# slp-rl/slamkit

Hardware: NVIDIA H100
Metric: speech-tokens/sec (SLAM seq=1024) (higher is better)
Workload: dtype bf16

## Files before the change

### slamkit_b200/csrc/gemm_tcgen05.cu

```cuda
#include "common.cuh"
#include <cudaTypedefs.h>
#include <stdio.h>
#include <mutex>
#include <type_traits>
#include <string.h>
#include <stdlib.h>
#include "kernels.h"
#include "../../include/slamkit_b200.h"

namespace {

constexpr int BM = 128;
constexpr int BK = 64;
constexpr int MMA_K = 16;
constexpr int GEMM_THREADS = 288;


struct GemmParams {
  int M, N, K;
  int batch;
  int a_mode;
  int passes;
  void* C;
  void* C_lo;
  int ldc;
  const void* bias;
  int bias_f32;
  const bf16* residual;
  const bf16* residual_lo;
  int ldr;
  int tiles_m, tiles_n;
  int out_f32;
  int round_before_res;
  int act;
  int col_gin, col_gout;
  int splits;
  float* splitk_ws;
  int tma_store;
  int reg_epi;
  int pdl;
  int sk_units;
  int sk_groups;
  int sk_G;
  int sk_colunits;
  int sk_carry;
  int units, n_groups;
  float* sk_ws;
  uint32_t* sk_flags;
  int epi;
  const bf16* aux;
  int ld_aux;
  const bf16* rope_cos;
  const bf16* rope_sin;
  const int* rope_pos;
  int rope_T, rope_cols, rope_maxpos, rope_rot;
};

template <int BN, int EW = 4>
struct GemmCfg {
  static constexpr int A_BYTES = BM * BK * 2;
  static constexpr int B_ATOMS = (BN + 63) / 64;
  static constexpr int B_BYTES = B_ATOMS * 64 * BK * 2;
  static constexpr int STAGE_BYTES = A_BYTES + B_BYTES;
  static constexpr int STAGES = (BN > 128) ? 4 : (BN > 64 ? 6 : 8);
  static constexpr int STAGING_BYTES = 4 * 2 * 4096;
  static constexpr int BAR_BYTES = 256;
  static constexpr int SMEM_BYTES = STAGES * STAGE_BYTES + STAGING_BYTES + BAR_BYTES + 1024;
  static_assert(BN % 64 == 0 || (BN == 224 && EW == 4), "a 32-column tail chunk only on the 224-wide tile");
  static_assert(STAGES * STAGE_BYTES >= BM * BN * 4, "the parked fp32 accumulator must fit in the stage ring");
  static_assert(SMEM_BYTES <= 227 * 1024, "sm_90 allows 227 KB of shared memory per block");
};

template <int BN>
SK_DEVINL uint32_t acc_chunk_addr(uint32_t base, int row, int chunk) {
  return base + (uint32_t)row * (BN * 4) + (uint32_t)((chunk ^ (row & 7)) << 4);
}
template <int BN>
SK_DEVINL void acc_park(uint32_t base, const float (&d)[BN / 2], int wg, int warp_in_wg, int lane) {
  const int r0 = 64 * wg + 16 * warp_in_wg + (lane >> 2);
#pragma unroll
  for (int j = 0; j < BN / 8; ++j) {
    const int chunk = 2 * j + ((lane & 3) >> 1);
    const uint32_t off = (uint32_t)(lane & 1) * 8u;
    asm volatile("st.shared.v2.f32 [%0], {%1, %2};" ::"r"(acc_chunk_addr<BN>(base, r0, chunk) + off), "f"(d[4 * j]),
                 "f"(d[4 * j + 1]) : "memory");
    asm volatile("st.shared.v2.f32 [%0], {%1, %2};" ::"r"(acc_chunk_addr<BN>(base, r0 + 8, chunk) + off), "f"(d[4 * j + 2]),
                 "f"(d[4 * j + 3]) : "memory");
  }
}
template <int BN>
SK_DEVINL void acc_ld_32x32(uint32_t base, uint32_t ta, uint32_t (&r)[32]) {
  const int row = (int)(ta >> 16) + (int)(threadIdx.x & 31);
  const int c0 = (int)(ta & 0xffffu) >> 2;
#pragma unroll
  for (int i = 0; i < 8; ++i)
    asm volatile("ld.shared.v4.b32 {%0, %1, %2, %3}, [%4];"
                 : "=r"(r[4 * i]), "=r"(r[4 * i + 1]), "=r"(r[4 * i + 2]), "=r"(r[4 * i + 3])
                 : "r"(acc_chunk_addr<BN>(base, row, c0 + i)) : "memory");
}

SK_DEVINL uint32_t staging_addr(uint32_t sbuf, int lane, int j, bool tail) {
  return tail ? sbuf + (uint32_t)lane * 64u + (uint32_t)((j ^ ((lane >> 1) & 3)) << 4)
              : sbuf + (uint32_t)lane * 128u + (uint32_t)((j ^ (lane & 7)) << 4);
}

SK_DEVINL float gelu_erf(float y) {
  const float a = fabsf(y);
  float t;
  asm("rcp.approx.ftz.f32 %0, %1;" : "=f"(t) : "f"(fmaf(0.3275911f * 0.70710678118654752440f, a, 1.0f)));
  float s = fmaf(0.5f * 1.061405429f, t, 0.5f * -1.453152027f);
  s = fmaf(s, t, 0.5f * 1.421413741f);
  s = fmaf(s, t, 0.5f * -0.284496736f);
  s = fmaf(s, t, 0.5f * 0.254829592f);
  const float e = ex2_approx((y * y) * -0.72134752044448170368f);
  return fmaf(-a, (s * t) * e, fmaxf(y, 0.0f));
}

SK_DEVINL float gelu_exact(float x) { return x * 0.5f * (1.0f + erff(x * 0.70710678118654752440f)); }
SK_DEVINL float gelu_exact_grad(float x) {
  const float cdf = 0.5f * (1.0f + erff(x * 0.70710678118654752440f));
  const float pdf = expf(-0.5f * x * x) * 0.39894228040143267794f;
  return cdf + x * pdf;
}

SK_DEVINL void stmatrix_x4(uint32_t addr, uint32_t a, uint32_t b, uint32_t c, uint32_t d) {
  asm volatile("stmatrix.sync.aligned.m8n8.x4.shared.b16 [%0], {%1, %2, %3, %4};" ::"r"(addr), "r"(a), "r"(b), "r"(c),
               "r"(d) : "memory");
}

template <bool SK>
struct WorkIter {
  int num_kb, splits, kb_per_split, total_items, tiles_n;
  int G, colunits, carry, units, n_groups, sk_groups, grp, mem;
  long sk_total, sk_cur, sk_end;
  int next_unit, next_item;
  int tile, split, kb_begin, kb_end, role;
  long unit_end_it;
  SK_DEVINL WorkIter(const GemmParams& p, int num_kb_, int kb_per_split_, int total_items_) {
    num_kb = num_kb_;
    splits = p.splits;
    kb_per_split = kb_per_split_;
    total_items = total_items_;
    tiles_n = p.tiles_n;
    G = p.sk_G;
    colunits = p.sk_colunits;
    carry = p.sk_carry;
    units = p.units;
    n_groups = p.n_groups;
    sk_groups = p.sk_groups;
    tile = split = kb_begin = kb_end = role = 0;
    unit_end_it = 0;
    sk_total = sk_cur = sk_end = 0;
    next_item = (int)blockIdx.x;
    next_unit = 0;
    grp = mem = 0;
    if (SK && p.sk_units > 0) {
      grp = (int)blockIdx.x / G;
      mem = (int)blockIdx.x - grp * G;
      next_item = total_items;
      next_unit = grp < n_groups ? p.sk_units + grp : units;
      if (grp < sk_groups) {
        sk_total = (long)p.sk_units * num_kb;
        sk_cur = sk_total * grp / sk_groups;
        sk_end = sk_total * (grp + 1) / sk_groups;
      }
    }
  }
  SK_DEVINL int tile_of(int unit) const { return colunits ? mem * tiles_n + unit : unit * G + mem; }
  SK_DEVINL bool next() {
    if (SK && sk_cur < sk_end && carry) {
      const int unit = (int)((sk_end - 1) / num_kb);
      const long ustart = (long)unit * num_kb;
      const long b = sk_cur > ustart ? sk_cur : ustart;
      kb_begin = (int)(b - ustart);
      kb_end = (int)(sk_end - ustart);
      unit_end_it = ustart + num_kb;
      tile = tile_of(unit);
      split = 0;
      role = kb_begin != 0 ? 3 : (kb_end < num_kb ? 1 : 0);
      sk_end = b;
      return true;
    }
    if (SK && sk_cur < sk_end) {
      const int unit = (int)(sk_cur / num_kb);
      kb_begin = (int)(sk_cur - (long)unit * num_kb);
      unit_end_it = (long)(unit + 1) * num_kb;
      const long e = sk_end < unit_end_it ? sk_end : unit_end_it;
      kb_end = kb_begin + (int)(e - sk_cur);
      tile = tile_of(unit);
      split = 0;
      role = kb_begin != 0 ? 1 : (e < unit_end_it ? 2 : 0);
      sk_cur = e;
// ... 746 lines not shown
#pragma unroll
            for (int t = 0; t < 16; ++t) pk[t] = pack_bf16(__uint_as_float(r0[2 * t]), __uint_as_float(r0[2 * t + 1]));
            if constexpr (!tail) {
              acc_ld(taddr + c2 * 64 + 32, r1);
              if (SK && n_contrib > 0) sk_fixup_add(r1, p.sk_ws, c2 * 2 + 1, row_in_tile, first_contrib, w.G, n_contrib);
#pragma unroll
              for (int t = 0; t < 16; ++t) pk[16 + t] = pack_bf16(__uint_as_float(r1[2 * t]), __uint_as_float(r1[2 * t + 1]));
            }
            stage_store(&tmC, pk, n0 + c2 * 64, tail_c);
          });
        } else if (p.tma_store && !p.bias && !p.act && p.residual && !p.residual_lo && p.epi == 0) {
          for_chunks([&](auto tail_c, int c2) {
            constexpr bool tail = decltype(tail_c)::value;
            constexpr int nj = tail ? 4 : 8;
            const int col64 = n0 + c2 * 64;
            if (col64 >= p.N) return;
            uint4 rv[8];
            if (row_ok) {
              const bf16* rp = p.residual + row * p.ldr + col64;
#pragma unroll
              for (int j = 0; j < 8; ++j) rv[j] = (j < nj && col64 + 8 * j < p.N) ? ldg128(rp + 8 * j) : make_uint4(0u, 0u, 0u, 0u);
            } else {
#pragma unroll
              for (int j = 0; j < 8; ++j) rv[j] = make_uint4(0u, 0u, 0u, 0u);
            }
            uint32_t r0[32], r1[32], pk[32];
            acc_ld(taddr + c2 * 64, r0);
            if (SK && n_contrib > 0) sk_fixup_add(r0, p.sk_ws, c2 * 2, row_in_tile, first_contrib, w.G, n_contrib);
            if constexpr (!tail) {
              acc_ld(taddr + c2 * 64 + 32, r1);
              if (SK && n_contrib > 0) sk_fixup_add(r1, p.sk_ws, c2 * 2 + 1, row_in_tile, first_contrib, w.G, n_contrib);
            }
#pragma unroll
            for (int j = 0; j < nj; ++j) {
              const uint32_t* r = j < 4 ? r0 + 8 * j : r1 + 8 * (j - 4);
              const uint32_t rw[4] = {rv[j].x, rv[j].y, rv[j].z, rv[j].w};
#pragma unroll
              for (int e = 0; e < 4; ++e) {
                const float2 f = unpack_bf16(rw[e]);
                float a0 = __uint_as_float(r[2 * e]), a1 = __uint_as_float(r[2 * e + 1]);
                if (p.round_before_res) {
                  const float2 t = unpack_bf16(pack_bf16(a0, a1));
                  a0 = t.x; a1 = t.y;
                }
                pk[4 * j + e] = pack_bf16(a0 + f.x, a1 + f.y);
              }
            }
            stage_store(&tmC, pk, col64, tail_c);
          });
        } else if (p.tma_store) {
          for_chunks([&](auto tail_c, int c2) {
            constexpr bool tail = decltype(tail_c)::value;
            const uint32_t sbuf = staging_base + (EW == 4 ? (uint32_t)warp * 8192u + (store_cnt & 1u) * 4096u : (uint32_t)warp * 4096u);
            if (lane == 0) {
              if constexpr (EW == 4) tma_store_wait_read<1>(); else tma_store_wait_read<0>();
            }
            __syncwarp();
#pragma unroll
            for (int half = 0; half < (tail ? 1 : 2); ++half) {
              uint32_t r[32];
              acc_ld(taddr + c2 * 64 + half * 32, r);
              if (SK && n_contrib > 0) sk_fixup_add(r, p.sk_ws, c2 * 2 + half, row_in_tile, first_contrib, w.G, n_contrib);
#pragma unroll
              for (int g = 0; g < 4; ++g) {
                const int col = n0 + c2 * 64 + half * 32 + g * 8;
                float v[8];
#pragma unroll
                for (int i = 0; i < 8; ++i) v[i] = __uint_as_float(r[g * 8 + i]);
                if (col < p.N) {
                  epi_bias_act(v, p, col);
                  if (row_ok) epi_residual(v, p, row, col);
                }
                asm volatile("st.shared.v4.b32 [%0], {%1, %2, %3, %4};" ::"r"(staging_addr(sbuf, lane, half * 4 + g, tail)),
                             "r"(pack_bf16(v[0], v[1])), "r"(pack_bf16(v[2], v[3])), "r"(pack_bf16(v[4], v[5])),
                             "r"(pack_bf16(v[6], v[7]))
                             : "memory");
              }
            }
            fence_proxy_async();
            __syncwarp();
            if (lane == 0) {
              tma_store_2d(tail ? &tmAux : &tmC, sbuf, n0 + c2 * 64, m0 + q * 32);
              tma_store_commit();
            }
            ++store_cnt;
          });
        }
        else
#pragma unroll 1
        for (int c = chalf * (BN / 32 / CS); c < (chalf + 1) * (BN / 32 / CS); ++c) {
          uint32_t r[32];
          acc_ld(taddr + c * 32, r);
          if (SK && n_contrib > 0) sk_fixup_add(r, p.sk_ws, c, row_in_tile, first_contrib, w.G, n_contrib);
          const int col0 = n0 + c * 32;
          if (row_ok && col0 < p.N) {
#pragma unroll
            for (int g = 0; g < 4; ++g) {
              const int col = col0 + g * 8;
              if (col < p.N) {
                float v[8];
#pragma unroll
                for (int i = 0; i < 8; ++i) v[i] = __uint_as_float(r[g * 8 + i]);
                if (p.splits > 1) {
                  float* dst = p.splitk_ws + ((size_t)split_idx * p.M + row_in) * p.N + col;
                  *reinterpret_cast<float4*>(dst) = make_float4(v[0], v[1], v[2], v[3]);
                  *reinterpret_cast<float4*>(dst + 4) = make_float4(v[4], v[5], v[6], v[7]);
                  continue;
                }
                epi_bias_act(v, p, col);
                int ocol = col;
                if (p.col_gin > 0) {
                  const int gi = col / p.col_gin, ci = col - gi * p.col_gin;
                  if (ci >= p.col_gout) continue;
                  ocol = gi * p.col_gout + ci;
                }
                epi_residual(v, p, row, ocol);
                if (p.out_f32) {
                  float* dst = reinterpret_cast<float*>(p.C) + row * p.ldc + ocol;
                  *reinterpret_cast<float4*>(dst) = make_float4(v[0], v[1], v[2], v[3]);
                  *reinterpret_cast<float4*>(dst + 4) = make_float4(v[4], v[5], v[6], v[7]);
                } else {
                  uint4 o;
                  o.x = pack_bf16(v[0], v[1]);
                  o.y = pack_bf16(v[2], v[3]);
                  o.z = pack_bf16(v[4], v[5]);
                  o.w = pack_bf16(v[6], v[7]);
                  stg128(reinterpret_cast<bf16*>(p.C) + row * p.ldc + ocol, o);
                  if (p.C_lo) {
                    const float2 h0 = unpack_bf16(o.x), h1 = unpack_bf16(o.y), h2 = unpack_bf16(o.z), h3 = unpack_bf16(o.w);
                    uint4 l;
                    l.x = pack_bf16(v[0] - h0.x, v[1] - h0.y);
                    l.y = pack_bf16(v[2] - h1.x, v[3] - h1.y);
                    l.z = pack_bf16(v[4] - h2.x, v[5] - h2.y);
                    l.w = pack_bf16(v[6] - h3.x, v[7] - h3.y);
                    stg128(reinterpret_cast<bf16*>(p.C_lo) + row * p.ldc + ocol, l);
                  }
                }
              }
            }
          }
        }
        if (SK && w.role == 2) {
          __syncwarp();
          if (lane == 0)
            for (int i = 0; i < n_contrib; ++i) p.sk_flags[(first_contrib + i * w.G) * 4 + q] = 0u;
        }
      }
      release_acc();
    }
    if ((epi_warp || p.reg_epi) && p.tma_store && lane == 0) tma_store_wait<0>();
  }
}

__global__ void splitk_reduce_kernel(const float* __restrict__ ws, bf16* __restrict__ C, int M, int N, int ldc, int splits,
                                     int accumulate, int round_before_res) {
  griddep_launch();
  griddep_wait();
  const long total = (long)M * N / 8;
  for (long i = blockIdx.x * (long)blockDim.x + threadIdx.x; i < total; i += (long)gridDim.x * blockDim.x) {
    const long e = i * 8;
    const int m = (int)(e / N), n = (int)(e % N);
    float acc[8] = {0, 0, 0, 0, 0, 0, 0, 0};
    for (int s = 0; s < splits; ++s) {
      const float* src = ws + ((size_t)s * M + m) * N + n;
      const float4 a = *reinterpret_cast<const float4*>(src), b = *reinterpret_cast<const float4*>(src + 4);
      acc[0] += a.x; acc[1] += a.y; acc[2] += a.z; acc[3] += a.w;
      acc[4] += b.x; acc[5] += b.y; acc[6] += b.z; acc[7] += b.w;
    }
    bf16* dst = C + (size_t)m * ldc + n;
    if (accumulate) {
      const uint4 o = *reinterpret_cast<const uint4*>(dst);
      const uint32_t ow[4] = {o.x, o.y, o.z, o.w};
#pragma unroll
      for (int k = 0; k < 4; ++k) {
        const float2 f = unpack_bf16(ow[k]);
        acc[2 * k] = (round_before_res ? bf16_round(acc[2 * k]) : acc[2 * k]) + f.x;
        acc[2 * k + 1] = (round_before_res ? bf16_round(acc[2 * k + 1]) : acc[2 * k + 1]) + f.y;
      }
    }
    stg128(dst, make_uint4(pack_bf16(acc[0], acc[1]), pack_bf16(acc[2], acc[3]), pack_bf16(acc[4], acc[5]),
                           pack_bf16(acc[6], acc[7])));
  }
}

PFN_cuTensorMapEncodeTiled_v12000 g_encode = nullptr;
std::once_flag g_encode_once;

void load_encode() {
  void* fn = nullptr;
  cudaDriverEntryPointQueryResult qres;
  cudaError_t e = cudaGetDriverEntryPoint("cuTensorMapEncodeTiled", &fn, cudaEnableDefault, &qres);
  if (e == cudaSuccess && qres == cudaDriverEntryPointSuccess) g_encode = (PFN_cuTensorMapEncodeTiled_v12000)fn;
}

}

int sk_make_tmap_2d(CUtensorMap* out, const void* ptr, int elem_bytes, uint64_t inner, uint64_t outer, uint64_t ld,
                    uint32_t box_inner, uint32_t box_outer) {
  std::call_once(g_encode_once, load_encode);
  SK_REQUIRE(g_encode != nullptr, "cuTensorMapEncodeTiled driver entry point not available");
  SK_REQUIRE((reinterpret_cast<uintptr_t>(ptr) & 15) == 0, "TMA base pointer must be 16-byte aligned");
  SK_REQUIRE((ld * elem_bytes) % 16 == 0, "TMA row pitch must be a multiple of 16 bytes (ld=%llu)",
             (unsigned long long)ld);
  SK_REQUIRE(box_inner * elem_bytes == 128 || box_inner * elem_bytes == 64, "box inner extent must be 128 (or 64) bytes");
  cuuint64_t dims[2] = {inner, outer};
  cuuint64_t strides[1] = {ld * (uint64_t)elem_bytes};
  cuuint32_t box[2] = {box_inner, box_outer};
  cuuint32_t estr[2] = {1, 1};
  CUtensorMapDataType dt = elem_bytes == 2 ? CU_TENSOR_MAP_DATA_TYPE_BFLOAT16 : CU_TENSOR_MAP_DATA_TYPE_FLOAT32;
  CUresult r = g_encode(out, dt, 2, const_cast<void*>(ptr), dims, strides, box, estr, CU_TENSOR_MAP_INTERLEAVE_NONE,
                        box_inner * elem_bytes == 64 ? CU_TENSOR_MAP_SWIZZLE_64B : CU_TENSOR_MAP_SWIZZLE_128B,
                        CU_TENSOR_MAP_L2_PROMOTION_L2_256B,
                        CU_TENSOR_MAP_FLOAT_OOB_FILL_NONE);
  SK_REQUIRE(r == CUDA_SUCCESS, "cuTensorMapEncodeTiled failed with CUresult %d (inner=%llu outer=%llu ld=%llu)", (int)r,
             (unsigned long long)inner, (unsigned long long)outer, (unsigned long long)ld);
  return 0;
}

int sk_make_tmap_3d(CUtensorMap* out, const void* ptr, uint64_t inner, uint64_t rows, uint64_t batch, uint64_t row_stride,
                    uint64_t batch_stride, uint32_t box_rows) {
  std::call_once(g_encode_once, load_encode);
  SK_REQUIRE(g_encode != nullptr, "cuTensorMapEncodeTiled driver entry point not available");
  SK_REQUIRE((reinterpret_cast<uintptr_t>(ptr) & 15) == 0, "TMA base pointer must be 16-byte aligned");
  SK_REQUIRE((row_stride * 2) % 16 == 0 && (batch_stride * 2) % 16 == 0, "TMA strides must be multiples of 16 bytes");
  cuuint64_t dims[3] = {inner, rows, batch};
  cuuint64_t strides[2] = {row_stride * 2, batch_stride * 2};
  cuuint32_t box[3] = {64, box_rows, 1};
  cuuint32_t estr[3] = {1, 1, 1};
  CUresult r = g_encode(out, CU_TENSOR_MAP_DATA_TYPE_BFLOAT16, 3, const_cast<void*>(ptr), dims, strides, box, estr,
                        CU_TENSOR_MAP_INTERLEAVE_NONE, CU_TENSOR_MAP_SWIZZLE_128B, CU_TENSOR_MAP_L2_PROMOTION_L2_256B,
                        CU_TENSOR_MAP_FLOAT_OOB_FILL_NONE);
  SK_REQUIRE(r == CUDA_SUCCESS, "cuTensorMapEncodeTiled(3d) failed with CUresult %d", (int)r);
  return 0;
}

namespace {

template <int BN, bool A_MN, bool B_MN, bool SK, int EW = 4>
int launch_gemm(const CUtensorMap* tm, const GemmParams& p, int grid, cudaStream_t stream) {
  using Cfg = GemmCfg<BN, EW>;
  static bool attr_set = false;
  if (!attr_set) {
    SK_CUDA_CHECK(cudaFuncSetAttribute(gemm_wgmma_kernel<BN, A_MN, B_MN, SK, EW>, cudaFuncAttributeMaxDynamicSharedMemorySize,
                                       Cfg::SMEM_BYTES));
    attr_set = true;
  }
  sk_prof_begin(0, stream);
  cudaError_t lerr = sk_launch_pdl_if(p.pdl != 0, gemm_wgmma_kernel<BN, A_MN, B_MN, SK, EW>, dim3(grid), dim3(GEMM_THREADS), (size_t)Cfg::SMEM_BYTES, stream,
                                   tm[0], tm[1], tm[2], tm[3], tm[4], tm[5], p);
  sk_prof_end(stream);
  SK_CUDA_CHECK(lerr);
  SK_LAUNCH_CHECK();
  return 0;
}

template <int BN, bool SK, int EW = 4>
int dispatch_major(bool a_mn, bool b_mn, const CUtensorMap* tm, const GemmParams& p, int grid, cudaStream_t s) {
  if (!a_mn && !b_mn) return launch_gemm<BN, false, false, SK, EW>(tm, p, grid, s);
  if (!a_mn && b_mn) return launch_gemm<BN, false, true, SK, EW>(tm, p, grid, s);
  if (a_mn && !b_mn) return launch_gemm<BN, true, false, SK, EW>(tm, p, grid, s);
  return launch_gemm<BN, true, true, SK, EW>(tm, p, grid, s);
}

inline int tile_cost(int bn) { return bn >= 256 ? 100 : (bn > 128 ? 61 + (bn - 128) * 39 / 128 : (bn == 128 ? 61 : 54)); }

constexpr size_t SK_FLAG_BYTES = 4096;

}

size_t sk_gemm_ws_min_bytes(void) { return (size_t)sk_num_sms() * SK_SLOT_FLOATS * sizeof(float) + SK_FLAG_BYTES; }

int sk_pick_bn(int M, int N, int force_bn, bool fit_forced, bool fit, bool whole_heads) {
  if (force_bn == 64 || force_bn == 128 || force_bn == 256) return force_bn;
  if (fit_forced && (force_bn == 192 || (force_bn == 224 && !whole_heads))) return force_bn;
  const int nsm = sk_num_sms();
  auto cost = [&](int bn) {
    const long tiles = (long)((M + BM - 1) / BM) * ((N + bn - 1) / bn);
    return ((tiles + nsm - 1) / nsm) * tile_cost(bn);
  };
  int best = 256;
  long best_cost = cost(256);
  for (const int bn : {128, 64}) {
    if (cost(bn) * 100 < best_cost * 75) {
      best_cost = cost(bn);
      best = bn;
    }
  }
  if (best == 256 && fit && N % 256 != 0) {
    for (const int bn : {224, 192}) {
      if (!(whole_heads && bn % 64 != 0) && cost(bn) * 100 < best_cost * 95) {
        best_cost = cost(bn);
        best = bn;
      }
    }
  }
  return best;
}

namespace {

int plan_gemm(const SkGemmEx& g, GemmParams& p, int& BN, int& ew, int& grid) {
  SK_REQUIRE(g.M > 0 && g.N > 0 && g.K > 0 && g.batch >= 1, "gemm: empty problem M=%d N=%d K=%d batch=%d", g.M, g.N, g.K,
             g.batch);
  SK_REQUIRE(g.N % 8 == 0, "gemm: N must be a multiple of 8 (N=%d)", g.N);
  SK_REQUIRE(g.ldc % 8 == 0 && (g.residual == nullptr || g.ldr % 8 == 0), "gemm: ldc/ldr must be multiples of 8");
  SK_REQUIRE((reinterpret_cast<uintptr_t>(g.C) & 15) == 0, "gemm: C must be 16-byte aligned");
  SK_REQUIRE(((reinterpret_cast<uintptr_t>(g.A) | reinterpret_cast<uintptr_t>(g.B) | reinterpret_cast<uintptr_t>(g.A_lo) |
               reinterpret_cast<uintptr_t>(g.B_lo)) & 15) == 0,
             "gemm: A and B must be 16-byte aligned");
  SK_REQUIRE((reinterpret_cast<uintptr_t>(g.bias) & 15) == 0 && (reinterpret_cast<uintptr_t>(g.residual) & 15) == 0,
             "gemm: bias and residual must be 16-byte aligned");
  SK_REQUIRE(g.passes == 1 || (g.passes == 3 && g.A_lo && g.B_lo), "gemm: passes must be 1, or 3 with lo operands");
  SK_REQUIRE(g.act >= 0 && g.act <= 2, "gemm: act must be 0 (none), 1 (GELU) or 2 (ReLU), got %d", g.act);
  const bool use3d = g.a_rows > 0;
  SK_REQUIRE(!use3d || !g.a_mn, "gemm: a batched / windowed A operand must be K-major");
  SK_REQUIRE(g.a_mode == 0 || use3d, "gemm: a_mode 1 needs the 3-D A view");
  SK_REQUIRE(use3d || g.lda >= (g.a_mn ? g.M : g.K), "gemm: lda=%d is smaller than the %s of A", g.lda, g.a_mn ? "M" : "K");
  SK_REQUIRE(g.ldb >= (g.b_mn ? g.N : g.K), "gemm: ldb=%d is smaller than the %s of B", g.ldb, g.b_mn ? "N" : "K");
  if (g.col_gin == 0) {
    const int out_cols = g.epi == 2 ? 2 * g.N : g.N;
    SK_REQUIRE(g.ldc >= out_cols, "gemm: ldc=%d is smaller than the %d output columns", g.ldc, out_cols);
    SK_REQUIRE(g.residual == nullptr || g.ldr >= g.N, "gemm: ldr=%d is smaller than N=%d", g.ldr, g.N);
  }
  const int nsm = sk_num_sms();
  static const int sk_env = [] { const char* e = getenv("SK_STREAMK"); return e ? atoi(e) : 1; }();
  static const int sk_min_idle = [] { const char* e = getenv("SK_STREAMK_MIN_IDLE"); return e ? atoi(e) : 20; }();
  static const int sk_min_kb = [] { const char* e = getenv("SK_STREAMK_MIN_KB"); return e ? atoi(e) : 32; }();
  const bool sk_ok = sk_env != 0 && g.batch == 1 && !use3d && g.passes == 1 && g.a_mode == 0 && g.splitk_ws != nullptr &&
                     g.splitk_ws_bytes >= sk_gemm_ws_min_bytes();
  const size_t ws_data_bytes = g.splitk_ws_bytes > SK_FLAG_BYTES ? g.splitk_ws_bytes - SK_FLAG_BYTES : 0;
  const bool fit = g.passes == 1 && g.batch == 1 && !use3d && g.a_mode == 0 && g.epi != 1 && g.epi != 2 && g.epi != 4 &&
                   g.epi != 5;
  SK_REQUIRE((g.force_bn != 192 && g.force_bn != 224) || (fit && !(g.force_bn == 224 && g.epi == 3)),
             "gemm: force_bn=%d needs a one-pass 2-D problem (and whole 64-column heads for RoPE)", g.force_bn);
  BN = (g.a_mode == 1) ? 64
                       : sk_pick_bn(g.M * g.batch, g.N, (g.epi == 1 || g.epi == 2) ? 256 : g.force_bn, fit,
                                    fit && !sk_ok, g.epi == 3);
  memset(&p, 0, sizeof(p));
  p.M = g.M; p.N = g.N; p.K = g.K;
  p.batch = g.batch;
  p.a_mode = (g.a_mode & 1) | (use3d ? 2 : 0);
  p.passes = g.passes;
  p.C = g.C; p.C_lo = g.C_lo; p.ldc = g.ldc;
  p.bias = g.bias; p.bias_f32 = g.bias_f32;
  p.residual = reinterpret_cast<const bf16*>(g.residual);
  p.residual_lo = reinterpret_cast<const bf16*>(g.residual_lo);
  p.ldr = g.ldr;
  p.tiles_m = (g.M + BM - 1) / BM;
  p.tiles_n = (g.N + BN - 1) / BN;
  p.out_f32 = g.out_f32;
  p.round_before_res = g.round_before_res;
  p.act = g.act;
  p.col_gin = g.col_gin; p.col_gout = g.col_gout;
  p.pdl = g.pdl;
  const long tiles = (long)p.tiles_m * p.tiles_n * g.batch;
  p.splits = 1;
  p.splitk_ws = nullptr;
  const int num_kb = (g.K + BK - 1) / BK;
  static const int splitk_env = [] { const char* e = getenv("SK_SPLITK"); return e ? atoi(e) : 1; }();
  static const int sk_ranges = [] { const char* e = getenv("SK_STREAMK_RANGES"); return e ? atoi(e) : 4; }();
  if (splitk_env && g.splitk_ws && g.batch == 1 && g.passes == 1 && !g.out_f32 && !g.bias && !g.act && !g.C_lo && g.col_gin == 0 &&
      g.epi == 0 &&
      (g.residual == nullptr || g.residual == g.C) && tiles * 2 <= nsm && num_kb >= 16) {
    int sp = (int)(nsm / tiles);
    if (sp > 8) sp = 8;
    if (sp > num_kb / 4) sp = num_kb / 4;
    if ((size_t)sp * g.M * g.N * sizeof(float) > ws_data_bytes) sp = (int)(ws_data_bytes / ((size_t)g.M * g.N * sizeof(float)));
    if (sp >= 2) {
      const int per = (num_kb + sp - 1) / sp;
      sp = (num_kb + per - 1) / per;
    }
    if (sp >= 2) {
      p.splits = sp;
      p.splitk_ws = reinterpret_cast<float*>(g.splitk_ws);
    }
  }
  p.tma_store = (!g.out_f32 && !g.C_lo && g.col_gin == 0 && p.splits == 1 && g.batch == 1 && !use3d && (g.ldc * 2) % 16 == 0)
                    ? 1 : 0;
  p.epi = g.epi;
  p.aux = reinterpret_cast<const bf16*>(g.aux);
  p.ld_aux = g.ld_aux;
  p.rope_cos = reinterpret_cast<const bf16*>(g.rope_cos);
  p.rope_sin = reinterpret_cast<const bf16*>(g.rope_sin);
  p.rope_pos = g.rope_pos;
  p.rope_T = g.rope_T; p.rope_cols = g.rope_cols; p.rope_maxpos = g.rope_maxpos;
  p.rope_rot = g.rope_rot == 0 ? 64 : g.rope_rot;
  if (g.epi == 6) {
    SK_REQUIRE(g.passes == 1 && g.batch == 1 && !use3d && g.residual && g.aux && !g.residual_lo && !g.act && !g.out_f32 &&
                   !g.C_lo && g.col_gin == 0 && g.round_before_res && g.ld_aux >= g.N && g.ld_aux % 8 == 0 &&
                   (reinterpret_cast<uintptr_t>(g.aux) & 15) == 0,
               "gemm: two-residual epilogue needs a plain one-pass bf16 GEMM, both residuals (16-byte aligned, pitch >= N) and "
               "round_before_res");
  } else if (g.epi != 0) {
    SK_REQUIRE(p.tma_store && g.passes == 1 && !g.residual && !g.act && g.splitk_ws == nullptr,
               "gemm: fused epilogue %d needs the plain bf16 TMA-store path (no residual / activation / scratch)", g.epi);
    if (g.epi == 1) {
      SK_REQUIRE(BN == 256 && g.N % 256 == 0 && g.aux_out && g.ld_aux_out % 8 == 0 && !g.bias,
                 "gemm: SwiGLU-forward epilogue needs N = 2F with F %% 128 == 0 and an act output");
    } else if (g.epi == 2) {
      SK_REQUIRE(BN == 256 && g.N % 128 == 0 && g.aux && g.ld_aux % 8 == 0 && !g.bias,
                 "gemm: SwiGLU-backward epilogue needs N = F with F %% 128 == 0 and the saved gu activation");
    } else if (g.epi == 3) {
      SK_REQUIRE(g.rope_cos && g.rope_sin && g.rope_T > 0 && g.rope_maxpos > 0 && g.rope_cols % 64 == 0 && g.N % 64 == 0 &&
                     !g.bias_f32,
                 "gemm: RoPE epilogue needs cos/sin tables, 64-column heads and a bf16 bias");
      SK_REQUIRE(p.rope_rot == 16 || p.rope_rot == 32 || p.rope_rot == 64,
                 "gemm: RoPE epilogue rotary width rope_rot=%d is not supported (16, 32 or 64)", g.rope_rot);
    } else if (g.epi == 4) {
      SK_REQUIRE(BN % 64 == 0 && g.N % 64 == 0 && g.aux_out && g.ld_aux_out >= g.N && g.ld_aux_out % 8 == 0 && !g.bias_f32 &&
                     (reinterpret_cast<uintptr_t>(g.aux_out) & 15) == 0,
                 "gemm: GELU-forward epilogue needs N %% 64 == 0, an act output (pitch >= N) and a bf16 bias");
    } else if (g.epi == 5) {
      SK_REQUIRE(BN % 64 == 0 && g.N % 64 == 0 && g.aux && g.ld_aux >= g.N && g.ld_aux % 8 == 0 && !g.bias &&
                     (reinterpret_cast<uintptr_t>(g.aux) & 15) == 0,
                 "gemm: GELU-backward epilogue needs N %% 64 == 0, the saved pre-activation (pitch >= N) and no bias");
    } else {
      SK_REQUIRE(false, "gemm: unknown fused epilogue %d", g.epi);
    }
  }
  p.sk_G = 1;
  if (sk_ok && BN == 256 && p.splits == 1 && num_kb >= sk_min_kb && (p.tiles_n <= 8 || p.tiles_m <= 8)) {
    const int colunits = p.tiles_n <= 8 ? 0 : 1;
    const int G = colunits ? p.tiles_m : p.tiles_n;
    const int units = colunits ? p.tiles_n : p.tiles_m;
    const int n_groups = nsm / G;
    const int rem = units % n_groups;
    const long slots = ((long)(units + n_groups - 1) / n_groups) * n_groups;
    const bool multiwave = units > n_groups;
    if (n_groups >= 1 && rem != 0 && (slots - units) * 100 >= slots * sk_min_idle &&
        (!colunits || multiwave || sk_env >= 2)) {
      if (colunits && multiwave) {
        p.sk_units = rem + n_groups;
        p.sk_groups = n_groups;
        p.sk_carry = 1;
      } else {
        p.sk_units = rem;
        p.sk_groups = n_groups < rem * sk_ranges ? n_groups : rem * sk_ranges;
      }
      p.sk_G = G;
      p.sk_colunits = colunits;
      p.units = units;
      p.n_groups = n_groups;
      p.sk_ws = reinterpret_cast<float*>(g.splitk_ws);
      p.sk_flags = reinterpret_cast<uint32_t*>(reinterpret_cast<uint8_t*>(g.splitk_ws) + ws_data_bytes);
    }
  }
  const long work = tiles * p.splits;
  grid = p.sk_units > 0 ? p.n_groups * p.sk_G : (int)(work < nsm ? work : nsm);
  static const int ew_env = [] { const char* e = getenv("SK_GEMM_EW"); return e ? atoi(e) : 0; }();
  ew = (p.sk_units == 0 && BN == 256 && p.tma_store && (ew_env == 8 || (ew_env == 0 && (g.epi == 2 || g.epi == 3 || g.epi == 4 || g.epi == 5)))) ? 8 : 4;
  p.reg_epi = (p.tma_store && p.sk_units == 0 && ew == 4 && !g.bias && !g.act && !g.residual && (g.epi == 0 || g.epi == 1)) ? 1 : 0;
  return 0;
}

}

int sk_gemm_plan_ex(const SkGemmEx& g, SkGemmPlan* out) {
  GemmParams p;
  int BN = 0, ew = 0, grid = 0;
  const int rc = plan_gemm(g, p, BN, ew, grid);
  if (rc) return rc;
  out->bn = BN;
  out->epi_warps = ew;
  out->splits = p.splits;
  out->sk_units = p.sk_units;
  out->sk_groups = p.sk_groups;
  out->sk_G = p.sk_G;
  out->sk_colunits = p.sk_colunits;
  out->tma_store = p.tma_store;
  out->grid = grid;
  return 0;
}

int sk_gemm_ex_launch(const SkGemmEx& g, cudaStream_t stream) {
  GemmParams p;
  int BN = 0, ew = 0, grid = 0;
  const int rc0 = plan_gemm(g, p, BN, ew, grid);
  if (rc0) return rc0;
  const bool use3d = g.a_rows > 0;
  CUtensorMap tm[6];
  const void* As[2] = {g.A, g.passes == 3 ? g.A_lo : g.A};
  const void* Bs[2] = {g.B, g.passes == 3 ? g.B_lo : g.B};
  for (int i = 0; i < 2; ++i) {
    int rc;
    CUtensorMap* ta = &tm[i == 0 ? 0 : 2];
    CUtensorMap* tb = &tm[i == 0 ? 1 : 3];
    if (use3d) {
      rc = sk_make_tmap_3d(ta, As[i], (uint64_t)g.a_inner, (uint64_t)g.a_rows, (uint64_t)g.batch, (uint64_t)g.a_row_stride,
                           (uint64_t)g.a_batch_stride, BM);
    } else if (!g.a_mn) {
      rc = sk_make_tmap_2d(ta, As[i], 2, (uint64_t)g.K, (uint64_t)g.M, (uint64_t)g.lda, BK, BM);
    } else {
      rc = sk_make_tmap_2d(ta, As[i], 2, (uint64_t)g.M, (uint64_t)g.K, (uint64_t)g.lda, 64, BK);
    }
    if (rc) return rc;
    if (!g.b_mn) rc = sk_make_tmap_2d(tb, Bs[i], 2, (uint64_t)g.K, (uint64_t)g.N, (uint64_t)g.ldb, BK, (uint32_t)BN);
    else         rc = sk_make_tmap_2d(tb, Bs[i], 2, (uint64_t)g.N, (uint64_t)g.K, (uint64_t)g.ldb, 64, BK);
    if (rc) return rc;
  }
  tm[4] = tm[0];
  const uint32_t box_rows = p.reg_epi ? 16 : 32;
  if (p.tma_store) {
    const int rc2 = sk_make_tmap_2d(&tm[4], g.C, 2, (uint64_t)(g.epi == 2 ? 2 * g.N : g.N), (uint64_t)g.M, (uint64_t)g.ldc, 64, box_rows);
    if (rc2) return rc2;
  }
  tm[5] = tm[4];
  if (g.epi == 1) {
    const int rc3 = sk_make_tmap_2d(&tm[5], g.aux_out, 2, (uint64_t)g.N / 2, (uint64_t)g.M, (uint64_t)g.ld_aux_out, 64, box_rows);
    if (rc3) return rc3;
  } else if (g.epi == 4) {
    const int rc3 = sk_make_tmap_2d(&tm[5], g.aux_out, 2, (uint64_t)g.N, (uint64_t)g.M, (uint64_t)g.ld_aux_out, 64, 32);
    if (rc3) return rc3;
  } else if (p.tma_store && BN % 64 != 0) {
    const int rc3 = sk_make_tmap_2d(&tm[5], g.C, 2, (uint64_t)g.N, (uint64_t)g.M, (uint64_t)g.ldc, 32, box_rows);
    if (rc3) return rc3;
  }
  int rc;
  if (p.sk_units > 0) {
    rc = dispatch_major<256, true>(g.a_mn, g.b_mn, tm, p, grid, stream);
  } else if (ew == 8) {
    rc = dispatch_major<256, false, 8>(g.a_mn, g.b_mn, tm, p, grid, stream);
  } else {
    switch (BN) {
      case 256: rc = dispatch_major<256, false>(g.a_mn, g.b_mn, tm, p, grid, stream); break;
      case 224: rc = dispatch_major<224, false>(g.a_mn, g.b_mn, tm, p, grid, stream); break;
      case 192: rc = dispatch_major<192, false>(g.a_mn, g.b_mn, tm, p, grid, stream); break;
      case 128: rc = dispatch_major<128, false>(g.a_mn, g.b_mn, tm, p, grid, stream); break;
      default:  rc = dispatch_major<64, false>(g.a_mn, g.b_mn, tm, p, grid, stream); break;
    }
  }
  if (rc) return rc;
  if (p.splits > 1) {
    SK_REQUIRE(g.residual == nullptr || g.residual == g.C, "gemm: split-K supports only in-place accumulation");
    const long n8 = (long)g.M * g.N / 8;
    int blocks = (int)((n8 + 255) / 256);
    if (blocks > sk_num_sms() * 8) blocks = sk_num_sms() * 8;
    sk_prof_begin(0, stream);
    SK_CUDA_CHECK(sk_launch_pdl(splitk_reduce_kernel, dim3(blocks), dim3(256), (size_t)(0), stream, p.splitk_ws, reinterpret_cast<bf16*>(g.C), g.M, g.N, g.ldc, p.splits,
                                                     g.residual != nullptr, g.round_before_res));
    sk_prof_end(stream);
    SK_LAUNCH_CHECK();
  }
  return 0;
}

SkGemmEx sk_gemm_desc(int M, int N, int K, const void* A, int lda, int a_mn, const void* B, int ldb, int b_mn, void* C,
                      int ldc, int out_f32, const void* bias, const void* residual, int ldr, int round_before_res, int act,
                      int force_bn, void* splitk_ws, size_t splitk_ws_bytes) {
  SkGemmEx g;
  memset(&g, 0, sizeof(g));
  g.M = M; g.N = N; g.K = K; g.batch = 1; g.passes = 1;
  g.A = A; g.lda = lda; g.a_mn = a_mn;
  g.B = B; g.ldb = ldb; g.b_mn = b_mn;
  g.C = C; g.ldc = ldc; g.out_f32 = out_f32;
  g.bias = bias; g.residual = residual; g.ldr = ldr; g.round_before_res = round_before_res; g.act = act;
  g.force_bn = force_bn;
  g.pdl = 1;
  g.splitk_ws = splitk_ws;
  g.splitk_ws_bytes = splitk_ws_bytes;
  return g;
}
int sk_gemm_launch(int M, int N, int K, const void* A, int lda, int a_mn, const void* B, int ldb, int b_mn, void* C,
                   int ldc, int out_f32, const void* bias, const void* residual, int ldr, int round_before_res, int act,
                   int force_bn, cudaStream_t stream, void* splitk_ws, size_t splitk_ws_bytes) {
  return sk_gemm_ex_launch(sk_gemm_desc(M, N, K, A, lda, a_mn, B, ldb, b_mn, C, ldc, out_f32, bias, residual, ldr,
                                        round_before_res, act, force_bn, splitk_ws, splitk_ws_bytes),
                           stream);
}

int sk_linear_swiglu_fwd_launch(int M, int F, int K, const void* x, const void* Wgu, void* gu, void* act, cudaStream_t s) {
  SkGemmEx g;
  memset(&g, 0, sizeof(g));
  g.M = M; g.N = 2 * F; g.K = K; g.batch = 1; g.passes = 1;
  g.A = x; g.lda = K; g.B = Wgu; g.ldb = K;
  g.C = gu; g.ldc = 2 * F;
  g.epi = 1; g.aux_out = act; g.ld_aux_out = F;
  g.pdl = 1;
  return sk_gemm_ex_launch(g, s);
}
int sk_linear_swiglu_bwd_launch(int M, int N, int F, const void* dy, const void* Wd, const void* gu, void* dgu, cudaStream_t s) {
  SkGemmEx g;
  memset(&g, 0, sizeof(g));
  g.M = M; g.N = F; g.K = N; g.batch = 1; g.passes = 1;
  g.A = dy; g.lda = N; g.B = Wd; g.ldb = F; g.b_mn = 1;
  g.C = dgu; g.ldc = 2 * F;
  g.epi = 2; g.aux = gu; g.ld_aux = 2 * F;
  g.pdl = 1;
  return sk_gemm_ex_launch(g, s);
}
int sk_linear_rope_launch(int M, int N, int K, const void* x, const void* W, const void* bias, void* out, const void* cos_t,
                          const void* sin_t, const int32_t* pos_ids, int T, int rope_cols, int max_positions, cudaStream_t s,
                          int rope_rot) {
  SkGemmEx g;
  memset(&g, 0, sizeof(g));
  g.M = M; g.N = N; g.K = K; g.batch = 1; g.passes = 1;
  g.A = x; g.lda = K; g.B = W; g.ldb = K;
  g.C = out; g.ldc = N;
  g.bias = bias;
  g.epi = 3; g.rope_cos = cos_t; g.rope_sin = sin_t; g.rope_pos = pos_ids; g.rope_T = T;
  g.rope_cols = rope_cols; g.rope_maxpos = max_positions; g.rope_rot = rope_rot;
  g.pdl = 1;
  return sk_gemm_ex_launch(g, s);
}
int sk_linear_gelu_fwd_launch(int M, int F, int K, const void* x, const void* W1, const void* b1, void* pre, void* act,
                              cudaStream_t s) {
  SkGemmEx g;
  memset(&g, 0, sizeof(g));
  g.M = M; g.N = F; g.K = K; g.batch = 1; g.passes = 1;
  g.A = x; g.lda = K; g.B = W1; g.ldb = K;
  g.C = pre; g.ldc = F;
  g.bias = b1;
  g.epi = 4; g.aux_out = act; g.ld_aux_out = F;
  g.pdl = 1;
  return sk_gemm_ex_launch(g, s);
}
int sk_linear_gelu_bwd_launch(int M, int N, int F, const void* dy, const void* W2, const void* pre, void* dpre, cudaStream_t s) {
  SkGemmEx g;
  memset(&g, 0, sizeof(g));
  g.M = M; g.N = F; g.K = N; g.batch = 1; g.passes = 1;
  g.A = dy; g.lda = N; g.B = W2; g.ldb = F; g.b_mn = 1;
  g.C = dpre; g.ldc = F;
  g.epi = 5; g.aux = pre; g.ld_aux = F;
  g.pdl = 1;
  return sk_gemm_ex_launch(g, s);
}
int sk_linear_res2_launch(int M, int N, int K, const void* x, const void* W, const void* bias, const void* res2, const void* res,
                          void* out, cudaStream_t s, void* splitk_ws, size_t splitk_ws_bytes) {
  SkGemmEx g = sk_gemm_desc(M, N, K, x, K, 0, W, K, 0, out, N, 0, bias, res, N, 1, 0, 0, splitk_ws, splitk_ws_bytes);
  g.epi = 6; g.aux = res2; g.ld_aux = N;
  return sk_gemm_ex_launch(g, s);
}
```

Baseline: 166,600.

## Add warp-specialized handoff GEMM kernel overlapping SwiGLU epilogue with next tile's mainloop

Adds a new persistent GEMM kernel in which two consumer warpgroups run wgmma, stage the bf16 tile into a dedicated swizzled shared-memory handoff buffer via stmatrix, and three separate epilogue warps apply the SwiGLU forward or backward epilogue while the MMA warps proceed to the next tile. It is selected for BN=256 single-pass non-split GEMMs with epi 1 or 2. The intent is to hide epilogue cost behind the mainloop. In exchange, the handoff buffer reduces pipeline stages to at most four, the kernel uses 384 threads, and the added barrier traffic could stall MMA warps if the epilogue is slower than the mainloop.

```diff
diff --git a/slamkit_b200/csrc/gemm_tcgen05.cu b/slamkit_b200/csrc/gemm_tcgen05.cu
--- a/slamkit_b200/csrc/gemm_tcgen05.cu
+++ b/slamkit_b200/csrc/gemm_tcgen05.cu
@@ -38,6 +38,7 @@
   float* splitk_ws;
   int tma_store;
   int reg_epi;
+  int ho;
   int pdl;
   int sk_units;
   int sk_groups;
@@ -1090,6 +1091,258 @@
   }
 }
 
+constexpr int HO_THREADS = 384;
+
+template <int BN>
+struct HandoffCfg {
+  static constexpr int A_BYTES = BM * BK * 2;
+  static constexpr int B_ATOMS = (BN + 63) / 64;
+  static constexpr int B_BYTES = B_ATOMS * 64 * BK * 2;
+  static constexpr int STAGE_BYTES = A_BYTES + B_BYTES;
+  static constexpr int HO_BYTES = BM * BN * 2;
+  static constexpr int BAR_BYTES = 256;
+  static constexpr int FIT = (227 * 1024 - HO_BYTES - BAR_BYTES - 1024) / STAGE_BYTES;
+  static constexpr int STAGES = FIT < 4 ? FIT : 4;
+  static constexpr int SMEM_BYTES = STAGES * STAGE_BYTES + HO_BYTES + BAR_BYTES + 1024;
+  static_assert(STAGES >= 3, "the handoff tile leaves at least three stages");
+  static_assert(BN == 256, "the SwiGLU epilogues take [128 gate | 128 up] column blocks");
+};
+
+template <int BN, bool A_MN, bool B_MN>
+__global__ void __launch_bounds__(HO_THREADS, 1)
+gemm_handoff_kernel(const __grid_constant__ CUtensorMap tmA, const __grid_constant__ CUtensorMap tmB,
+                    const __grid_constant__ CUtensorMap tmC, const __grid_constant__ CUtensorMap tmAux, GemmParams p) {
+  using Cfg = HandoffCfg<BN>;
+  constexpr int NC64 = BN / 64;
+  griddep_launch();
+  extern __shared__ uint8_t smem_raw[];
+  const uint32_t smem_base = (smem_u32(smem_raw) + 1023u) & ~1023u;
+  const uint32_t ho_base = smem_base + Cfg::STAGES * Cfg::STAGE_BYTES;
+  const uint32_t bar_base = ho_base + Cfg::HO_BYTES;
+  auto full_bar = [&](int s) { return bar_base + 8u * s; };
+  auto empty_bar = [&](int s) { return bar_base + 8u * (Cfg::STAGES + s); };
+  const uint32_t ho_full = bar_base + 8u * (2 * Cfg::STAGES);
+  const uint32_t ho_empty = ho_full + 8u;
+  auto ho_addr = [&](int c, int row, int j) -> uint32_t {
+    return ho_base + (uint32_t)c * 16384u + (uint32_t)row * 128u + (uint32_t)((j ^ (row & 7)) << 4);
+  };
+
+  const int warp = threadIdx.x >> 5;
+  const int lane = threadIdx.x & 31;
+  const int total_items = p.tiles_m * p.tiles_n;
+  const int num_kb = (p.K + BK - 1) / BK;
+  constexpr uint32_t STAGE_TX = Cfg::A_BYTES + (B_MN ? Cfg::B_ATOMS * 64 * BK * 2 : BN * BK * 2);
+
+  if (threadIdx.x == 0) {
+    tma_prefetch_desc(&tmA);
+    tma_prefetch_desc(&tmB);
+    for (int s = 0; s < Cfg::STAGES; ++s) {
+      mbar_init(full_bar(s), 1);
+      mbar_init(empty_bar(s), 8);
+    }
+    mbar_init(ho_full, 8);
+    mbar_init(ho_empty, 3);
+    fence_mbar_init();
+  }
+  __syncthreads();
+  griddep_wait();
+
+  if (warp == 8) {
+    if (lane == 0) {
+      int stage = 0;
+      uint32_t phase = 0;
+      WorkIter<false> w(p, num_kb, num_kb, total_items);
+      while (w.next()) {
+        const int m0 = (w.tile / p.tiles_n) * BM;
+        const int n0 = (w.tile % p.tiles_n) * BN;
+        for (int kb = 0; kb < num_kb; ++kb) {
+          mbar_wait_nocall(empty_bar(stage), phase ^ 1u);
+          const uint32_t fb = full_bar(stage);
+          mbar_arrive_expect_tx(fb, STAGE_TX);
+          const uint32_t sA = smem_base + stage * Cfg::STAGE_BYTES;
+          const uint32_t sB = sA + Cfg::A_BYTES;
+          if (!A_MN) {
+            tma_load_2d(sA, &tmA, fb, kb * BK, m0);
+          } else {
+#pragma unroll
+            for (int j = 0; j < BM / 64; ++j) tma_load_2d(sA + j * (BK * 128), &tmA, fb, m0 + 64 * j, kb * BK);
+          }
+          if (!B_MN) {
+            tma_load_2d(sB, &tmB, fb, kb * BK, n0);
+          } else {
+#pragma unroll
+            for (int j = 0; j < Cfg::B_ATOMS; ++j) tma_load_2d(sB + j * (BK * 128), &tmB, fb, n0 + 64 * j, kb * BK);
+          }
+          if (++stage == Cfg::STAGES) { stage = 0; phase ^= 1u; }
+        }
+      }
+    }
+  } else if (warp < 8) {
+    const int wg = warp >> 2;
+    int stage = 0;
+    uint32_t phase = 0;
+    uint32_t t = 0;
+    WorkIter<false> w(p, num_kb, num_kb, total_items);
+    while (w.next()) {
+      float acc[BN / 2];
+#pragma unroll
+      for (int i = 0; i < BN / 2; ++i) acc[i] = 0.f;
+      int prev = -1;
+      for (int kb = 0; kb < num_kb; ++kb) {
+        mbar_wait_nocall(full_bar(stage), phase);
+        wgmma_fence();
+        const uint32_t sA = smem_base + stage * Cfg::STAGE_BYTES + (uint32_t)wg * 8192u;
+        const uint32_t sB = smem_base + stage * Cfg::STAGE_BYTES + Cfg::A_BYTES;
+#pragma unroll
+        for (int k = 0; k < BK / MMA_K; ++k) {
+          const uint64_t adesc = A_MN ? gmma_desc_sw128(sA + k * (MMA_K * 128), BK * 128, 1024)
+                                      : gmma_desc_sw128(sA + k * (MMA_K * 2), 16, 1024);
+          const uint64_t bdesc = B_MN ? gmma_desc_sw128(sB + k * (MMA_K * 128), BK * 128, 1024)
+                                      : gmma_desc_sw128(sB + k * (MMA_K * 2), 16, 1024);
+          wgmma_bf16<BN, A_MN ? 1 : 0, B_MN ? 1 : 0>(acc, adesc, bdesc);
+        }
+        wgmma_commit();
+        wgmma_wait<1>();
+        if (prev >= 0 && lane == 0) mbar_arrive(empty_bar(prev));
+        prev = stage;
+        if (++stage == Cfg::STAGES) { stage = 0; phase ^= 1u; }
+      }
+      wgmma_wait<0>();
+      if (prev >= 0 && lane == 0) mbar_arrive(empty_bar(prev));
+      if (t > 0) mbar_wait_nocall(ho_empty, (t - 1) & 1u);
+      const int srow = 16 * warp + (lane & 7) + (lane & 8);
+#pragma unroll
+      for (int c2 = 0; c2 < NC64; ++c2) {
+#pragma unroll
+        for (int jj = 0; jj < 8; jj += 2) {
+          const int j0 = 8 * c2 + jj, j1 = j0 + 1;
+          stmatrix_x4(ho_addr(c2, srow, jj + (lane >> 4)), pack_bf16(acc[4 * j0], acc[4 * j0 + 1]),
+                      pack_bf16(acc[4 * j0 + 2], acc[4 * j0 + 3]), pack_bf16(acc[4 * j1], acc[4 * j1 + 1]),
+                      pack_bf16(acc[4 * j1 + 2], acc[4 * j1 + 3]));
+        }
+      }
+      fence_proxy_async();
+      __syncwarp();
+      if (lane == 0) mbar_arrive(ho_full);
+      ++t;
+    }
+  } else {
+    const int e = warp - 9;
+    constexpr int NU = 4 * NC64;
+    uint32_t t = 0;
+    WorkIter<false> w(p, num_kb, num_kb, total_items);
+    const int lpiece = lane & 7, lrsub = lane >> 3;
+    const size_t row4_in = (size_t)4 * p.ld_aux * sizeof(bf16), row4_out = (size_t)4 * p.ldc * sizeof(bf16);
+    auto piece_off = [&](int m0, int n0, int u, size_t ld) -> size_t {
+      const int acol = n0 + (u >> 2) * 64;
+      const int gcol = (acol >> 7) * 256 + (acol & 127) + lpiece * 8;
+      return ((size_t)(m0 + (u & 3) * 32 + lrsub) * ld + gcol) * sizeof(bf16);
+    };
+    uint4 gv[8], uv[8];
+    auto gu_load_k = [&](int k, int m0, int n0, int u) {
+      if (u < NU && m0 + (u & 3) * 32 + 4 * k + lrsub < p.M && n0 + (u >> 2) * 64 < p.N) {
+        const uint8_t* base = reinterpret_cast<const uint8_t*>(p.aux) + piece_off(m0, n0, u, (size_t)p.ld_aux);
+        gv[k] = ldg128(base + k * row4_in);
+        uv[k] = ldg128(base + k * row4_in + 256);
+      } else {
+        gv[k] = make_uint4(0u, 0u, 0u, 0u);
+        uv[k] = make_uint4(0u, 0u, 0u, 0u);
+      }
+    };
+    while (w.next()) {
+      const int m0 = (w.tile / p.tiles_n) * BM;
+      const int n0 = (w.tile % p.tiles_n) * BN;
+      if (p.epi == 2) {
+#pragma unroll
+        for (int k = 0; k < 8; ++k) gu_load_k(k, m0, n0, e);
+      }
+      mbar_wait_nocall(ho_full, t & 1u);
+      if (p.epi == 2) {
+        if constexpr (BN == 256) {
+#pragma unroll 1
+          for (int u = e; u < NU; u += 3) {
+            const int c2 = u >> 2, q = u & 3;
+            const bool col_ok = n0 + c2 * 64 < p.N;
+            uint8_t* obase = reinterpret_cast<uint8_t*>(p.C) + piece_off(m0, n0, u, (size_t)p.ldc);
+#pragma unroll
+            for (int k = 0; k < 8; ++k) {
+              const int rr2 = 4 * k + lrsub;
+              uint32_t dw[4];
+              asm volatile("ld.shared.v4.b32 {%0, %1, %2, %3}, [%4];"
+                           : "=r"(dw[0]), "=r"(dw[1]), "=r"(dw[2]), "=r"(dw[3]) : "r"(ho_addr(c2, q * 32 + rr2, lpiece)));
+              const uint32_t gw[4] = {gv[k].x, gv[k].y, gv[k].z, gv[k].w}, uw[4] = {uv[k].x, uv[k].y, uv[k].z, uv[k].w};
+              if (u + 3 < NU) gu_load_k(k, m0, n0, u + 3);
+              uint32_t og[4], ou[4];
+#pragma unroll
+              for (int i = 0; i < 4; ++i) {
+                const float2 gf = unpack_bf16(gw[i]);
+                const float s0 = sigmoid_f(gf.x), s1 = sigmoid_f(gf.y);
+                const uint32_t sil2 = pack_bf16(gf.x * s0, gf.y * s1);
+                const float ds0 = s0 * (1.0f + gf.x * (1.0f - s0)), ds1 = s1 * (1.0f + gf.y * (1.0f - s1));
+                const bf162 d2 = *reinterpret_cast<const bf162*>(&dw[i]);
+                bf162 du2 = __hmul2(d2, *reinterpret_cast<const bf162*>(&uw[i]));
+                bf162 o2 = __hmul2(d2, *reinterpret_cast<const bf162*>(&sil2));
+                const float2 duf = __bfloat1622float2(du2);
+                og[i] = pack_bf16(duf.x * ds0, duf.y * ds1);
+                ou[i] = *reinterpret_cast<uint32_t*>(&o2);
+              }
+              if (col_ok && m0 + q * 32 + rr2 < p.M) {
+                stg128(obase + k * row4_out, make_uint4(og[0], og[1], og[2], og[3]));
+                stg128(obase + k * row4_out + 256, make_uint4(ou[0], ou[1], ou[2], ou[3]));
+              }
+            }
+          }
+        }
+      } else if (p.epi == 1) {
+        if constexpr (BN == 256) {
+#pragma unroll 1
+          for (int u = e; u < 8; u += 3) {
+            const int i = u >> 2, q = u & 3;
+            if (lane == 0) {
+              tma_store_2d(&tmC, ho_addr(i, q * 32, 0), n0 + 64 * i, m0 + q * 32);
+              tma_store_2d(&tmC, ho_addr(2 + i, q * 32, 0), n0 + 128 + 64 * i, m0 + q * 32);
+              tma_store_commit();
+            }
+            const int row = q * 32 + lane;
+            uint32_t pk[32];
+#pragma unroll
+            for (int j = 0; j < 8; ++j) {
+              uint32_t g[4], uu[4];
+              asm volatile("ld.shared.v4.b32 {%0, %1, %2, %3}, [%4];"
+                           : "=r"(g[0]), "=r"(g[1]), "=r"(g[2]), "=r"(g[3]) : "r"(ho_addr(i, row, j)));
+              asm volatile("ld.shared.v4.b32 {%0, %1, %2, %3}, [%4];"
+                           : "=r"(uu[0]), "=r"(uu[1]), "=r"(uu[2]), "=r"(uu[3]) : "r"(ho_addr(2 + i, row, j)));
+#pragma unroll
+              for (int x = 0; x < 4; ++x) {
+                const float2 gf = unpack_bf16(g[x]), uf = unpack_bf16(uu[x]);
+                const float2 sb = unpack_bf16(pack_bf16(silu_f(gf.x), silu_f(gf.y)));
+                pk[4 * j + x] = pack_bf16(sb.x * uf.x, sb.y * uf.y);
+              }
+            }
+            if (lane == 0) tma_store_wait_read<0>();
+            __syncwarp();
+#pragma unroll
+            for (int j = 0; j < 8; ++j)
+              asm volatile("st.shared.v4.b32 [%0], {%1, %2, %3, %4};" ::"r"(ho_addr(i, row, j)), "r"(pk[4 * j]),
+                           "r"(pk[4 * j + 1]), "r"(pk[4 * j + 2]), "r"(pk[4 * j + 3]) : "memory");
+            fence_proxy_async();
+            __syncwarp();
+            if (lane == 0) {
+              tma_store_2d(&tmAux, ho_addr(i, q * 32, 0), (n0 >> 1) + 64 * i, m0 + q * 32);
+              tma_store_commit();
+            }
+          }
+        }
+      }
+      if (lane == 0) tma_store_wait_read<0>();
+      __syncwarp();
+      if (lane == 0) mbar_arrive(ho_empty);
+      ++t;
+    }
+    if (lane == 0) tma_store_wait<0>();
+  }
+}
+
 __global__ void splitk_reduce_kernel(const float* __restrict__ ws, bf16* __restrict__ C, int M, int N, int ldc, int splits,
                                      int accumulate, int round_before_res) {
   griddep_launch();
@@ -1186,6 +1439,24 @@
   sk_prof_begin(0, stream);
   cudaError_t lerr = sk_launch_pdl_if(p.pdl != 0, gemm_wgmma_kernel<BN, A_MN, B_MN, SK, EW>, dim3(grid), dim3(GEMM_THREADS), (size_t)Cfg::SMEM_BYTES, stream,
                                    tm[0], tm[1], tm[2], tm[3], tm[4], tm[5], p);
+  sk_prof_end(stream);
+  SK_CUDA_CHECK(lerr);
+  SK_LAUNCH_CHECK();
+  return 0;
+}
+
+template <int BN, bool A_MN, bool B_MN>
+int launch_handoff(const CUtensorMap* tm, const GemmParams& p, int grid, cudaStream_t stream) {
+  using Cfg = HandoffCfg<BN>;
+  static bool attr_set = false;
+  if (!attr_set) {
+    SK_CUDA_CHECK(cudaFuncSetAttribute(gemm_handoff_kernel<BN, A_MN, B_MN>, cudaFuncAttributeMaxDynamicSharedMemorySize,
+                                       Cfg::SMEM_BYTES));
+    attr_set = true;
+  }
+  sk_prof_begin(0, stream);
+  cudaError_t lerr = sk_launch_pdl_if(p.pdl != 0, gemm_handoff_kernel<BN, A_MN, B_MN>, dim3(grid), dim3(HO_THREADS),
+                                      (size_t)Cfg::SMEM_BYTES, stream, tm[0], tm[1], tm[4], tm[5], p);
   sk_prof_end(stream);
   SK_CUDA_CHECK(lerr);
   SK_LAUNCH_CHECK();
@@ -1387,7 +1658,8 @@
   grid = p.sk_units > 0 ? p.n_groups * p.sk_G : (int)(work < nsm ? work : nsm);
   static const int ew_env = [] { const char* e = getenv("SK_GEMM_EW"); return e ? atoi(e) : 0; }();
   ew = (p.sk_units == 0 && BN == 256 && p.tma_store && (ew_env == 8 || (ew_env == 0 && (g.epi == 2 || g.epi == 3 || g.epi == 4 || g.epi == 5)))) ? 8 : 4;
-  p.reg_epi = (p.tma_store && p.sk_units == 0 && ew == 4 && !g.bias && !g.act && !g.residual && (g.epi == 0 || g.epi == 1)) ? 1 : 0;
+  p.ho = (ew_env != 8 && p.tma_store && p.sk_units == 0 && g.passes == 1 && !g.a_mn && BN == 256 && (g.epi == 1 || g.epi == 2)) ? 1 : 0;
+  p.reg_epi = (!p.ho && p.tma_store && p.sk_units == 0 && ew == 4 && !g.bias && !g.act && !g.residual && (g.epi == 0 || g.epi == 1)) ? 1 : 0;
   return 0;
 }
 
@@ -1454,7 +1726,9 @@
     if (rc3) return rc3;
   }
   int rc;
-  if (p.sk_units > 0) {
+  if (p.ho) {
+    rc = g.b_mn ? launch_handoff<256, false, true>(tm, p, grid, stream) : launch_handoff<256, false, false>(tm, p, grid, stream);
+  } else if (p.sk_units > 0) {
     rc = dispatch_major<256, true>(g.a_mn, g.b_mn, tm, p, grid, stream);
   } else if (ew == 8) {
     rc = dispatch_major<256, false, 8>(g.a_mn, g.b_mn, tm, p, grid, stream);
```

Result: no change. 167,700, median of 6 (+0.6%).
